# tturturiello/lightweight-snappy

Measured on AMD Instinct MI355X. Metric: compress + decompress MB/s at 1/2/4/8 MI355X; % HBM roofline; ratio vs ref, higher is better.
Workload: dtype u8

## Files before the change

### lightweight-snappy_amd/csrc/snappy_kernels.hip

```cpp
#include <hip/hip_runtime.h>
#include <stdint.h>
#include <type_traits>

#include "snappy_kernels.h"

#ifndef SNAPPY_TU
#define SNAPPY_TU 0
#endif
#define SNAPPY_TU_COMPRESS (SNAPPY_TU != 2)
#define SNAPPY_TU_DECODE (SNAPPY_TU != 1)

#if ((defined(SNAPPY_K2_NOLIT) && SNAPPY_K2_NOLIT) || defined(SNAPPY_K4_NOFAR)) && !defined(SNAPPY_MEASUREMENT_BUILD)
#error "SNAPPY_K2_NOLIT / SNAPPY_K4_NOFAR write wrong output: measurement builds only (-DSNAPPY_MEASUREMENT_BUILD)"
#endif

namespace snappy_amd {

__device__ int amdgcn_writelane(int val, int lanesel, int old) __asm("llvm.amdgcn.writelane.i32");


constexpr uint32_t kTable = 4096;
constexpr uint32_t kMul = 0x1e35a7bdu;

typedef uint32_t u32x4 __attribute__((ext_vector_type(4)));
// ... 390 lines not shown
    })

    uint32_t T = 256, lg = 8;
    while (T < kTable && T < L) { T <<= 1; lg++; }
    const uint32_t shift = 32 - lg;

    const uint32_t cur0 = __builtin_amdgcn_readfirstlane(REG_OF(0));
    const uint32_t init = TAG_OF(cur0) << 16;
    for (uint32_t i = lane; i < kTable; i += 64) TBL_WRITE(i, init);
    __syncthreads();

    uint32_t *tok = reinterpret_cast<uint32_t *>(tokens) + (uint64_t)u * tok_cap;
    uint32_t *tok_full = reinterpret_cast<uint32_t *>(tokens) + ((uint64_t)gridDim.x + u) * tok_cap;
    uint32_t tka = 0, tkb = 0;
    uint32_t nt = 0, pend = 0;
    uint32_t acc = 0, cend = 0;
    if (hdr_mode == SNAPPY_HDR_EVERY_UNIT) acc = varint_len(L);
    else if (hdr_mode == SNAPPY_HDR_FIRST_UNIT && u == 0) acc = varint_len(header_value);
    uint32_t *const segu = seg_off + 2 * (uint64_t)u * segs;
    auto flush_tokens = [&]() {
        const bool has = lane < pend;
        const uint32_t pos = tka & 0xFFFF, len = tka >> 16, end = pos + len;
        const uint32_t prev = (uint32_t)__builtin_amdgcn_update_dpp((int)cend, (int)end, 0x138, 0xF, 0xF, false);
        const uint32_t litn = pos - prev;
        if (has) {
            const uint32_t lc = len - 4 < 255 ? len - 4 : 255u, gc = litn < 255 ? litn : 255u;
            tok[nt + lane] = tkb | (lc << 16) | (gc << 24);
            if (lc == 255 || gc == 255) tok_full[nt + lane] = litn | (len << 16);
        }
        const uint32_t b = has ? (litn ? literal_bytes(litn) : 0u) + copy_bytes(len, tkb) : 0u;
        uint32_t tot;
        const uint32_t ex = wave_excl_scan(b, lane, &tot);
        if (has && ((nt + lane) & (kK2Seg - 1)) == 0)
            *reinterpret_cast<uint2 *>(segu + 2 * ((nt + lane) / kK2Seg)) = make_uint2(acc + ex, prev);
        if (pend) cend = __builtin_amdgcn_readlane(end, pend - 1);
        acc += tot;
        nt += pend;
        pend = 0;
    };

    uint32_t q0 = 0, d0 = 0, dr = 0, dv = 0, bv = 0, hv = 0;
    uint32_t pdl1 = 0, pdc = 0;
    uint16_t ent = 0;
    uint8_t ent_t = 0;
    uint32_t adr = 0, word = 0;
    uint32_t pdnz = 0;
    uint64_t m_win = 0, m_win17 = 0;
    bool lsw = false;
#ifndef SNAPPY_K1R_WIN_ALIGN
#define SNAPPY_K1R_WIN_ALIGN 1
#endif
#define WINDOW_AT(qq)                                                                              \
    do {                                                                                           \
        q0 = (qq);                                                                                 \
        ring_to((q0 >> 8) + 2, std::true_type{});     \
        d0 = q0 >> 2;                                                                              \
        dr = d0 & 63;                                                                              \
        {                                                                                          \
            uint32_t _r0, _r1;                                                                     \
            REG_PAIR(d0 >> 6, _r0, _r1);                                                           \
            dv = lane >= dr ? _r0 : _r1;                                                           \
        }                                                                                          \
        if (SNAPPY_K1R_WIN_ALIGN == 2 || (SNAPPY_K1R_WIN_ALIGN && !BIG)) { \
                          \
                                \
            const uint32_t _p = q0 + lane;                                                          \
            const uint32_t _k = (_p - 1) >> 2;                        \
            const uint32_t _a = (uint32_t)__builtin_amdgcn_ds_bpermute((int)(_k << 2), (int)dv);   \
            const uint32_t _b = (uint32_t)__builtin_amdgcn_ds_bpermute((int)((_k + 1) << 2), (int)dv); \
            bv = __builtin_amdgcn_alignbit(_a, _b, 0u - (_p << 3));                                  \
        } else {                                                                                   \
            const uint32_t _k = d0 + (((q0 & 3) + lane) >> 2);      \
            const uint32_t _a = (uint32_t)__builtin_amdgcn_ds_bpermute((int)(_k << 2), (int)dv);   \
            const uint32_t _b = (uint32_t)__builtin_amdgcn_ds_bpermute((int)((_k + 1) << 2), (int)dv); \
            bv = funnel_bytes(_a, _b, perm_sel((q0 + lane) & 3));                                 \
        }                                                                                          \
        {                                                                                          \
            const uint32_t _pr = bv * kMul;                                                        \
            hv = (_pr >> shift) | (__builtin_amdgcn_ubfe(_pr, shift - 8, 8) << 16);                \
        }                                                                                          \
    } while (0)
#define WINDOW_LS(qq)                                                                              \
    do {                                                                                           \
        WINDOW_AT(qq);                                                                             \
        adr = TBL_ADR(hv & 0xFFFF);                                                                \
        TBL_READ_ENT(adr);                              \
                          \
        const uint32_t _best = nearest_same_key<DMAX>(__builtin_amdgcn_alignbit(hv, hv, 16) + 0x10000u); \
        const bool _has = _best < 65536u;                                                          \
        const uint32_t _pd = _has ? _best >> 8 : 0u;                                               \
              \
        pdl1 = _has ? lane - _pd + 1 - (_pd == 1 ? 1u : 0u) : 0xFFFFFF00u;  \
        pdc = q0 + lane - _pd;                                                                     \
        pdnz = _best & 0xFFu;              \
                   \
        const int32_t _w16 = (int32_t)(L - 16 - q0), _w17 = (int32_t)(L - 17 - q0);              \
        const bool _inw = (int32_t)lane <= _w16 && lane <= 62;                                     \
        m_win = __ballot(_inw);                                                                    \
        m_win17 = __ballot((int32_t)lane <= _w17 && lane <= 62);                                   \
        word = (q0 + lane) | (hv & 0xFF0000u);                                                     \
        if (!_inw) word |= 1u << 24;    \
        lsw = true;                                                      \
    } while (0)

    auto match_len_from = [&](uint32_t pf, uint32_t cand, uint32_t len) -> uint32_t {
            for (;;) {
                if (pf + len >= L) break;
                const uint32_t qa = pf + len, qb = cand + len;
                ring_to((qa >> 8) + 2, std::false_type{});
                const uint32_t a0 = DW_LANES(qa >> 2), b0 = CAND_LANES(qb >> 2);
                const uint32_t va = funnel_bytes(a0, wave_shl1(a0), perm_sel(qa & 3));
                const uint32_t vb = funnel_bytes(b0, wave_shl1(b0), perm_sel(qb & 3));
                const uint32_t yy = lane < 63 ? (va ^ vb) : 0;
                const uint64_t bb = __ballot(yy != 0);
                if (bb) {
                    const uint32_t m = (uint32_t)__builtin_ctzll(bb);
                    len += 4 * m + ((uint32_t)__builtin_clz(__builtin_amdgcn_readlane(yy, m)) >> 3);
                    break;
                }
                len += 252;
            }
        return len;
    };
    auto match_len = [&](uint32_t pf, uint32_t cand) -> uint32_t {
        const uint32_t pa = (uint32_t)__builtin_amdgcn_ds_bpermute((int)(((pf >> 2) + lane) << 2), (int)dv);
        const uint32_t ca = CAND_LANES(cand >> 2);
        const uint32_t pv = funnel_bytes(pa, wave_shl1(pa), perm_sel(pf & 3));
        const uint32_t cv = funnel_bytes(ca, wave_shl1(ca), perm_sel(cand & 3));
        const uint32_t y = pv ^ cv;
        const uint64_t bad = __ballot(y != 0) & 0xFFFFull;
        if (bad) {
            const uint32_t m = (uint32_t)__builtin_ctzll(bad);
            return 4 * m + ((uint32_t)__builtin_clz(__builtin_amdgcn_readlane(y, m)) >> 3);
        }
        return match_len_from(pf, cand, 64);
    };
    auto put_token = [&](uint32_t pf, uint32_t len, uint32_t off) {
        tka = (uint32_t)amdgcn_writelane((int)(pf | (len << 16)), (int)pend, (int)tka);
        tkb = (uint32_t)amdgcn_writelane((int)off, (int)pend, (int)tkb);
        pend++;
    };
    uint32_t dka = 0, dkb = 0, dkn = 0;
    auto drain_token = [&]() {
        tka = (uint32_t)amdgcn_writelane((int)dka, (int)pend, (int)tka);
        tkb = (uint32_t)amdgcn_writelane((int)dkb, (int)pend, (int)tkb);
        pend += dkn;
        dkn = 0;
    };

#ifdef SNAPPY_K1R_RSTAMPS
    const uint64_t t_loop = clock64();
    uint64_t rs_flush = 0, rs_win = 0, rs_asm = 0;
    uint32_t rs_n = 0, rs_nfl = 0, rs_nasm = 0, rs_code[6] = {0, 0, 0, 0, 0, 0};
#endif
#ifdef SNAPPY_K1R_STATS
    const uint64_t t_loop = clock64();
    uint32_t n_probe = 0, n_match = 0, n_round = 0, n_refresh = 0;
#endif

#if !defined(SNAPPY_K1R_STATS) && !defined(SNAPPY_K1R_LSTAMPS) && !defined(SNAPPY_K1R_CXX_ROUNDS)
#define K1R_ASM_ROUNDS 1
#else
#define K1R_ASM_ROUNDS 0
#endif
#if K1R_ASM_ROUNDS
#ifndef SNAPPY_K1R_PAD32
#define SNAPPY_K1R_PAD32 2
#endif
#ifndef SNAPPY_K1R_PAD64
#define SNAPPY_K1R_PAD64 0
#endif
#ifndef SNAPPY_K1R_PAD64A
#define SNAPPY_K1R_PAD64A -1
#endif
#ifndef SNAPPY_K1R64_HALF32
#define SNAPPY_K1R64_HALF32 1
#endif
#define K1R_STR2(x) #x
#define K1R_STR(x) K1R_STR2(x)
#define K1R_LOOP_PLACE(pad) ".if " K1R_STR(pad) " >= 0\n.p2align 6\n.rept " K1R_STR(pad) "\ns_nop 0\n.endr\n.endif\n"
#define K1R_CAND32 "s_lshr_b32 %[s0], %[c], 8\n\t"
#define K1R_CAND64                                                                                  \
    "s_cmp_lt_u32 %[c], %[seghi]\n\t"                                                              \
    "s_cbranch_scc1 L%=_far\n\t"                                                                   \
    "s_bfe_u32 %[s0], %[c], 0x70008\n\t"                                                           \
    "s_cmp_eq_u32 %[s0], 127\n\t"                                                                  \
    "s_cbranch_scc1 L%=_wrap\n\t"
#define K1R_SEGHI64(seg_hi) "s"(((seg_hi) - kRegs) << 8)
#define K1R_HIT_PREDTAG                                                                             \
    "v_cndmask_b32_sdwa %[t1], %[pdc], %[ent], vcc dst_sel:DWORD dst_unused:UNUSED_PAD "             \
    "src0_sel:DWORD src1_sel:WORD_0\n\t"                           \
    "v_cndmask_b32_e32 %[t0], %[pdnz], %[entt], vcc\n\t"                           \
    "v_cmp_eq_u32_sdwa %[hm], %[t0], %[word] src0_sel:DWORD src1_sel:WORD_1\n\t"
#define K1R_HIT32 K1R_HIT_PREDTAG
#define K1R_HIT64 K1R_HIT_PREDTAG
#define K1R_DRAIN                                                                                   \
    "s_mov_b32 m0, %[pend]\n\t"           \
    "v_writelane_b32 %[tka], %[dka], m0\n\t"                                                        \
    "v_writelane_b32 %[tkb], %[dkb], m0\n\t"                                                        \
    "s_add_u32 %[pend], %[pend], %[dkn]\n\t"
#define K1R_SKIPFIX "s_cmp_eq_u32 %[dkn], 0\n\ts_cselect_b32 %[skip], %[skip], 32\n\t"
#define K1R_INSERTS(cnt, lo)                                                                        \
    "s_bfm_b64 exec, " cnt ", " lo "\n\t"                                                          \
    "ds_write_b16 %[adr], %[word]\n\t"                                                              \
    "ds_write_b8_d16_hi %[adrt], %[word] offset:%[tagb]\n\t"                                        \
    "s_mov_b64 exec, %[sx]\n\t"                                                                     \
    "ds_read_u16 %[ent], %[adr]\n\t"                                   \
    "ds_read_u8 %[entt], %[adrt] offset:%[tagb]\n\t"
#ifndef SNAPPY_K1R_X45
#define SNAPPY_K1R_X45 1
#endif
#if SNAPPY_K1R_X45
#define K1R_LENCHECK                                                                                \
    "v_readlane_b32 %[s0], %[t2], %[s1]\n\t"                                                        \
    "s_add_u32 %[s2], %[s0], -4\n\t"                                                                \
    "s_cmp_gt_u32 %[s2], 59\n\t"                                                                    \
    "s_cbranch_scc1 L%=_x4\n\t"
#define K1R_X4 "s_cmp_lt_u32 %[s0], 4\n\ts_cbranch_scc1 L%=_x5\n\ts_mov_b32 %[code], 4\n\ts_branch L%=_end\n"
#else
#define K1R_LENCHECK                                                                                \
    "s_cmp_gt_u32 %[s1], 15\n\t"                                                                    \
    "s_cbranch_scc1 L%=_x4\n\t"                                                                    \
    "v_readlane_b32 %[s0], %[t2], %[s1]\n\t"                                                       \
    "s_cmp_lt_u32 %[s0], 4\n\t"            \
    "s_cbranch_scc1 L%=_x5\n\t"
#define K1R_X4 "s_mov_b32 %[code], 4\n\ts_branch L%=_end\n"
#endif
#define K1R_NOHIT_TAIL(T)                                                                           \
    "s_cmp_gt_u32 %[skip], %[lsmax]\n\t"                                                           \
    "s_cbranch_scc1 L%=_x1\n\t"                                                                    \
    "s_cmp_gt_u32 %[p], %[lm16]\n\t"                                                               \
    "s_cbranch_scc1 L%=_x1\n\t"                                                                    \
    "s_cmp_gt_u32 %[lane0], %[l0max]\n\t"                                                          \
    "s_cbranch_scc1 L%=_x2\n\t"                                                                    \
    "s_cmp_le_u32 %[skip], %[skipmax]\n\t"                                                         \
    "s_cbranch_scc1 L%=_top" T "\n"
#ifndef SNAPPY_K1R_EARLY_DK
#define SNAPPY_K1R_EARLY_DK 1
#endif
#if SNAPPY_K1R_EARLY_DK
#define K1R_DK_EARLY "s_sub_u32 %[dkb], %[pf], %[c]\n\t"
#define K1R_DK_LATE "s_mov_b32 %[dkn], 1\n\t"
#else
#define K1R_DK_EARLY
#define K1R_DK_LATE "s_sub_u32 %[dkb], %[pf], %[c]\n\ts_mov_b32 %[dkn], 1\n\t"
#endif
#define K1R_ROUND_BODY(CAND, HIT, T)                                                                \
            "L%=_top" T ":\n\t"                                                                          \
            "s_lshl_b64 %[valid], %[dmask], %[lane0]\n\t"                                           \
            "v_cmp_gt_i32_e32 vcc, %[lane0], %[pdl1]\n\t"                   \
            "s_waitcnt lgkmcnt(0)\n\t"                                                              \
            HIT                                                                                     \
            "s_and_b64 %[hm], %[hm], %[valid]\n\t"                                                  \
            "s_cbranch_scc0 L%=_nohit" T "\n\t"                                      \
            "s_ff1_i32_b64 %[f], %[hm]\n\t"                                                         \
            "v_readlane_b32 %[c], %[t1], %[f]\n\t"                                                  \
            "s_add_u32 %[pf], %[q0], %[f]\n\t"                                                      \
            "v_add3_u32 %[t2], %[pf], -1, %[lane4]\n\t"               \
            "ds_bpermute_b32 %[t2], %[t2], %[dv]\n\t"                         \
            CAND                                                                                    \
            "s_bfe_u32 %[s1], %[c], 0x60002\n\t"                                                    \
            "v_cmp_le_u32_e32 vcc, %[s1], %[lane]\n\t"            \
            "v_add_u32_e32 %[t1], %[c], %[lane4]\n\t"                                               \
            "s_set_gpr_idx_on %[s0], gpr_idx(SRC0,SRC1)\n\t"                                        \
            "v_cndmask_b32_e32 %[t3], v3, v2, vcc\n\t"                                              \
            "s_set_gpr_idx_off\n\t"                                                                 \
            "ds_bpermute_b32 %[t3], %[t1], %[t3]\n\t"                          \
            "L%=_farret" T ":\n\t"                                                                       \
            K1R_DRAIN                          \
            K1R_DK_EARLY                                                                            \
            "s_cmp_lt_u32 %[lane0], %[f]\n\t"                                                       \
            "s_subb_u32 %[s0], %[lane0], 0\n\t"                                            \
            "v_mul_i32_i24_e64 %[t0], %[pf], -8\n\t"                         \
            "s_sub_u32 %[s2], %[f], %[s0]\n\t"                                                      \
            "s_add_u32 %[s2], %[s2], 1\n\t"                              \
            "s_and_b32 %[s3], %[c], 3\n\t"                                                          \
            "s_mul_i32 %[s3], %[s3], 0xfefefeff\n\t"                                                \
            "s_add_i32 %[s3], %[s3], 0x7060504\n\t"                         \
            "s_waitcnt lgkmcnt(0)\n\t"                                                \
            "v_mov_b32_dpp %[t1], %[t2] wave_shl:1 row_mask:0xf bank_mask:0xf bound_ctrl:1\n\t"     \
            "v_mov_b32_dpp %[t4], %[t3] wave_shl:1 row_mask:0xf bank_mask:0xf bound_ctrl:1\n\t"     \
            "v_alignbit_b32 %[t2], %[t2], %[t1], %[t0]\n\t"                                         \
            "v_perm_b32 %[t3], %[t3], %[t4], %[s3]\n\t"                                             \
            K1R_INSERTS("%[s2]", "%[s0]")                                                           \
            "v_cmp_ne_u32_e32 vcc, %[t2], %[t3]\n\t"                                                \
            "v_xor_b32_e32 %[t2], %[t2], %[t3]\n\t"                                                 \
            "v_ffbh_u32_e32 %[t2], %[t2]\n\t"                                                       \
            "v_bfe_u32 %[t2], %[t2], 3, 2\n\t"                                                      \
            "v_lshl_or_b32 %[t2], %[lane], 2, %[t2]\n\t"  \
            "s_ff1_i32_b32 %[s1], vcc_lo\n\t"                                                       \
            K1R_LENCHECK                                                                            \
            "s_add_u32 %[lane0], %[f], %[s0]\n\t"                                                   \
            "s_pack_ll_b32_b16 %[dka], %[pf], %[s0]\n\t"                                           \
            K1R_DK_LATE                                                                             \
            "s_cmp_le_i32 %[lane0], %[lim0]\n\t"          \
            "s_cbranch_scc1 L%=_top" T "\n\t"                                                            \
            "s_sub_u32 %[s2], %[L], %[pf]\n\t"  \
            "s_min_u32 %[s0], %[s0], %[s2]\n\t"                                                     \
            "s_add_u32 %[p], %[pf], %[s0]\n\t"                                                      \
            "s_sub_u32 %[lane0], %[p], %[q0]\n\t"                                                   \
            "s_lshl_b32 %[s1], %[s0], 16\n\t"                                                       \
            "s_or_b32 %[dka], %[s1], %[pf]\n\t"                                                     \
            "s_cmp_gt_u32 %[p], %[lm16]\n\t"                                                        \
            "s_cbranch_scc1 L%=_x1\n\t"                                                             \
            "s_branch L%=_x2\n"                                                                     \
            "L%=_nohit" T ":\n\t"                                                                        \
            K1R_SKIPFIX                                                                             \
            "s_and_b64 %[valid], %[valid], %[mwin]\n\t"                                             \
            "s_bcnt1_i32_b64 %[s0], %[valid]\n\t"  \
            K1R_DRAIN                                                                               \
            "s_mov_b32 %[dkn], 0\n\t"                                                               \
            "s_add_i32 %[s1], %[lane0], -1\n\t"                                                     \
            "s_add_u32 %[s2], %[skip], %[s0]\n\t"                                                   \
            "s_add_i32 %[s3], %[s2], -1\n\t"                                                        \
            "s_add_u32 %[c], %[s0], 1\n\t"                           \
            K1R_INSERTS("%[c]", "%[s1]")                     \
            "s_lshr_b32 %[s3], %[s3], 5\n\t"              \
            "s_add_u32 %[lane0], %[s1], %[s0]\n\t"           \
            "s_add_u32 %[lane0], %[lane0], %[s3]\n\t"                                               \
            "s_add_u32 %[p], %[q0], %[lane0]\n\t"                                                   \
            "s_mov_b32 %[skip], %[s2]\n\t"                                                          \
            K1R_NOHIT_TAIL(T)
#if SNAPPY_K1R64_HALF32
#define K1R64_HALF_SEL "s_cmp_eq_u32 %[seghi], 0\n\ts_cbranch_scc1 L%=_topa\n"
#define K1R64_HALF_LOOP "s_branch L%=_x3\n" K1R_LOOP_PLACE(SNAPPY_K1R_PAD64A) K1R_ROUND_BODY(K1R_CAND32, K1R_HIT64, "a")
#else
#define K1R64_HALF_SEL ""
#define K1R64_HALF_LOOP ""
#endif
#define K1R_ASM_ROUNDS_STMT(code, fx, cx, e32, et32, CAND, SEGHI, HIT, PAD, DUAL_SEL, DUAL_LOOP)    \
    do {                                                                                            \
        uint32_t _m0s, _pf, _s0, _s1, _s2, _s3, _t0, _t1, _t2, _t3, _t4;                            \
        uint64_t _valid, _hm;                                                                       \
        asm volatile(                                                                               \
            "s_mov_b32 %[m0s], m0\n\t"                                                              \
            "s_cmp_gt_u32 %[skip], %[skipmax]\n\t"    \
            "s_cbranch_scc1 L%=_x3\n"                                                               \
            DUAL_SEL                                                                                \
            K1R_LOOP_PLACE(PAD)                                                                     \
            K1R_ROUND_BODY(CAND, HIT, "")                                                           \
            DUAL_LOOP                                                                               \
            "L%=_x3:\n\ts_mov_b32 %[code], 3\n\ts_branch L%=_end\n"                                 \
            "L%=_x1:\n\ts_mov_b32 %[code], 1\n\ts_branch L%=_end\n"                                 \
            "L%=_x2:\n\ts_mov_b32 %[code], 2\n\ts_branch L%=_end\n"                                 \
            "L%=_x4:\n\t" K1R_X4                                                                   \
            "L%=_far:\n\t"                     \
            "s_and_b32 %[s1], %[c], -4\n\t"                                                         \
            "v_add_u32_e32 %[t1], %[s1], %[lane4]\n\t"                                              \
            "global_load_dword %[t3], %[t1], %[srcb]\n\t"                                           \
            "s_mov_b32 %[s1], 0x10203\n\t"                                                          \
            "s_waitcnt vmcnt(0)\n\t"                                                                \
            "v_perm_b32 %[t3], %[t3], %[t3], %[s1]\n\t"     \
            "s_branch L%=_farret\n"                                                                 \
            "L%=_wrap:\n\t"                \
            "s_bfe_u32 %[s1], %[c], 0x60002\n\t"                                                    \
            "v_cmp_le_u32_e32 vcc, %[s1], %[lane]\n\t"                                              \
            "v_add_u32_e32 %[t1], %[c], %[lane4]\n\t"                                               \
            "s_nop 0\n\t"                                                                            \
            "v_cndmask_b32_e32 %[t3], v2, v129, vcc\n\t"                                            \
            "ds_bpermute_b32 %[t3], %[t1], %[t3]\n\t"                                               \
            "s_branch L%=_farret\n"                                                                 \
            "L%=_x5:\n\ts_mov_b32 %[code], 5\n"                                                     \
            "L%=_end:\n\t"                                                                          \
            K1R_SKIPFIX                                                                             \
            "s_mov_b32 m0, %[m0s]\n\t"                                                              \
            "s_waitcnt lgkmcnt(0)"                                                                  \
            : [p] "+s"(p), [skip] "+s"(skip), [lane0] "+s"(lane0), [pend] "+s"(pend), [dka] "+s"(dka), \
              [dkb] "+s"(dkb), [dkn] "+s"(dkn), [code] "=&s"(code), [f] "=&s"(fx),                     \
              [c] "=&s"(cx),                                                                        \
              [m0s] "=&s"(_m0s), [pf] "=&s"(_pf), [s0] "=&s"(_s0), [s1] "=&s"(_s1), [s2] "=&s"(_s2),   \
              [s3] "=&s"(_s3), [valid] "=&s"(_valid), [hm] "=&s"(_hm), [ent] "+v"(e32),                \
              [entt] "+v"(et32), [tka] "+v"(tka), [tkb] "+v"(tkb), [t0] "=&v"(_t0), [t1] "=&v"(_t1),  \
              [t2] "=&v"(_t2), [t3] "=&v"(_t3), [t4] "=&v"(_t4)                                        \
            : [q0] "s"(q0), [L] "s"(L), [lm16] "s"(L - 16), [mwin] "s"(m_win), [seghi] SEGHI,         \
              [lim0] "s"(__builtin_elementwise_min((int32_t)(62 - SNAPPY_K1R_RMIN), (int32_t)L - 16 - (int32_t)q0)), \
              [dv] "v"(dv),                                                                         \
              [pdl1] "v"(pdl1), [pdc] "v"(pdc), [pdnz] "v"(pdnz), [adr] "v"(adr), [adrt] "v"(adr >> 1), \
              [word] "v"(word), [lane] "v"(lane), [lane4] "v"(lane << 2), [srcb] "s"(src),            \
              [sx] "s"(__builtin_amdgcn_read_exec()),      \
              [skipmax] "i"(64 - DMAX), [dmask] "i"((1u << DMAX) - 1), [lsmax] "i"(64 - SNAPPY_K1R_LSMIN), \
              [l0max] "i"(62 - SNAPPY_K1R_RMIN), [tagb] "i"(kTagBase), "{v[2:33]}"(g0), "{v[34:65]}"(g1), \
              "{v[66:97]}"(g2), "{v[98:129]}"(g3)                                                      \
            : "vcc", "scc", "memory");                                                              \
    } while (0)
#endif
#if defined(SNAPPY_K1R_LSTAMPS)
    uint64_t seg[6] = {0, 0, 0, 0, 0, 0};
    uint64_t s0, s1, s2, s3, s4, s5, s6;
#endif
    uint32_t p = 1, skip = 33;
    while (!(L - p < (skip >> 5) + 15)) {
#ifdef SNAPPY_K1R_STATS
        n_round++;
#endif
        if (skip <= 64 - SNAPPY_K1R_LSMIN) {
            auto refresh = [&]() {
                LSTAMP(s5);
#ifdef SNAPPY_K1R_STATS
                n_refresh++;
#endif
#ifdef SNAPPY_K1R_RSTAMPS
                uint64_t r0, r1, r2;
                const bool rfl = pend + dkn > 48;
                if constexpr (BIG) {
                    RSTAMP(r0);
                    WINDOW_LS(p - 1);
                    RSTAMP(r1);
                    if (rfl) flush_tokens();
                    RSTAMP(r2);
                    rs_win += r1 - r0;
                    rs_flush += r2 - r1;
                } else {
                    RSTAMP(r0);
                    if (rfl) flush_tokens();
                    RSTAMP(r1);
                    WINDOW_LS(p - 1);
                    RSTAMP(r2);
                    rs_flush += r1 - r0;
                    rs_win += r2 - r1;
                }
                rs_n++;
                rs_nfl += rfl;
                if (false)
#endif
                if constexpr (BIG) {
                    const bool fl = pend + dkn > 48;
                    WINDOW_LS(p - 1);
                    if (fl) flush_tokens();
                } else
                {
                    if (pend + dkn > 48) flush_tokens();
                    WINDOW_LS(p - 1);
                }
                LSTAMP(s6);
                LSEG(5, s5, s6);
            };
            uint32_t lane0 = p - q0;
            bool went = false;
            if (!lsw || lane0 + SNAPPY_K1R_RMIN > 62) {
                refresh();
                lane0 = 1;
                went = true;
            }
            if (!went) TBL_READ_ENT(adr);
            for (;;) {
#if K1R_ASM_ROUNDS
                {
                    uint32_t code, fx, cx;
                    uint32_t e32 = ent, et32 = ent_t;
#ifdef SNAPPY_K1R_RSTAMPS
                    uint64_t ra0, ra1;
                    RSTAMP(ra0);
#endif
                    if constexpr (BIG)
                        K1R_ASM_ROUNDS_STMT(code, fx, cx, e32, et32, K1R_CAND64, K1R_SEGHI64(seg_hi), K1R_HIT64, SNAPPY_K1R_PAD64,
                                            K1R64_HALF_SEL, K1R64_HALF_LOOP);
                    else
                        K1R_ASM_ROUNDS_STMT(code, fx, cx, e32, et32, K1R_CAND32, "i"(0), K1R_HIT32, SNAPPY_K1R_PAD32, "", "");
#ifdef SNAPPY_K1R_RSTAMPS
                    RSTAMP(ra1);
                    rs_asm += ra1 - ra0;
                    rs_nasm++;
                    rs_code[code < 6 ? code : 0]++;
#endif
                    ent = (uint16_t)e32;
                    ent_t = (uint8_t)et32;
                    if (code == 1) break;
                    if (code == 2) {
                        refresh();
                        lane0 = 1;
                        continue;
                    }
                    if (code >= 4) {
                        const uint32_t f = fx, pf = q0 + fx, c = cx;
                        uint32_t np;
                        if (code == 4) {
                            uint32_t len = __builtin_elementwise_min(match_len_from(pf, c, 64), L - pf);
                            dka = pf | (len << 16);
                            dkb = pf - c;
                            dkn = 1;
                            np = pf + len;
                            skip = 32;
                        } else {
                            dkn = 0;
                            if (f == lane0) {
                                TBL_INSERT(lane - (lane0 - 1) <= 1);
                                LDS_ORDER();
                                TBL_READ_ENT(adr);
                            }
                            np = pf + ((skip + f - lane0) >> 5);
                            skip += f - lane0 + 1;
                        }
                        p = np;
                        if (!(skip <= 64 - SNAPPY_K1R_LSMIN && p <= L - 16)) break;
                        lane0 = p - q0;
                        if (lane0 + SNAPPY_K1R_RMIN > 62) {
                            refresh();
                            lane0 = 1;
                        }
                        continue;
                    }
                }
#endif
                LSTAMP(s0);
                drain_token();
                uint64_t valid = (((1ull << DMAX) - 1) << lane0) & m_win;
                if (__builtin_expect(skip > 64 - DMAX, 0)) {
                    const uint32_t kcap = 64 - skip;
                    valid = ((2ull << kcap) - 1) << lane0;
                    if (lane0 + kcap < 64) valid &= ~((1ull << (lane0 + kcap)) & ~m_win17);
                    valid &= m_win;
                }
                const bool inr = (int32_t)pdl1 >= (int32_t)lane0;
                const uint32_t hitnz = (inr ? pdnz : (uint32_t)ent_t) ^ ((word >> 16) & 0xFFu);
                const uint64_t hm = __ballot(hitnz == 0) & valid;
                const uint32_t candv = inr ? pdc : ent;
                const uint32_t f = (uint32_t)__builtin_ctzll(hm);
                LSTAMP(s1);
                LSEG(0, s0, s1);
                uint32_t np;
                if (__builtin_expect(hm != 0, 1)) {
                    const uint32_t pf = q0 + f;
                    const uint32_t c = __builtin_amdgcn_readlane(candv, f) & 0xFFFF;
                    const uint32_t pa = (uint32_t)__builtin_amdgcn_ds_bpermute(
                        (int)(((pf >> 2) + lane) << 2), (int)dv);
                    const uint32_t ca = CAND_LANES(c >> 2);
                    __builtin_amdgcn_sched_barrier(0);
                    const uint32_t lo0 = f > lane0 ? lane0 - 1 : lane0;
                    TBL_INSERT(lane - lo0 <= f - lo0);
                    LDS_ORDER();
                    TBL_READ_ENT(adr);
                    LSTAMP(s2);
                    LSEG(1, s1, s2);
                    const uint32_t pv = funnel_bytes(pa, wave_shl1(pa), perm_sel(pf & 3));
                    const uint32_t cv = funnel_bytes(ca, wave_shl1(ca), perm_sel(c & 3));
                    const uint32_t y = pv ^ cv;
                    const uint64_t bad = __ballot(y != 0) & 0xFFFFull;
                    const uint32_t lenv = 4 * lane + ((uint32_t)__builtin_clz(y | 1) >> 3);
                    uint32_t len = __builtin_amdgcn_readlane(lenv, (uint32_t)__builtin_ctzll(bad) & 63);
                    if (__builtin_expect(bad == 0, 0)) len = match_len_from(pf, c, 64);
                    LSTAMP(s3);
                    LSEG(2, s2, s3);
#ifdef SNAPPY_K1R_STATS
                    n_probe += f - lane0 + 1;
#endif
                    len = __builtin_elementwise_min(len, L - pf);
                    dka = pf | (len << 16);
                    dkb = pf - c;
                    if (__builtin_expect(len >= 4, 1)) {
#ifdef SNAPPY_K1R_STATS
                        n_match++;
#endif
                        dkn = 1;
                        np = pf + len;
                        skip = 32;
                    } else {
                        dkn = 0;
                        if (f == lane0) {
                            TBL_INSERT(lane - (lane0 - 1) <= 1);
                            LDS_ORDER();
                            TBL_READ_ENT(adr);
                        }
                        np = pf + ((skip + f - lane0) >> 5);
                        skip += f - lane0 + 1;
                    }
                } else {
                    LSTAMP(s3);
                    dka = dkb = dkn = 0;
                    const uint32_t nk = (uint32_t)__builtin_popcountll(valid);
                    TBL_INSERT(lane - (lane0 - 1) <= nk);
                    LDS_ORDER();
                    TBL_READ_ENT(adr);
                    np = q0 + lane0 + nk - 1 + ((skip + nk - 1) >> 5);
                    skip += nk;
#ifdef SNAPPY_K1R_STATS
                    n_probe += nk;
#endif
                }
                p = np;
                LSTAMP(s4);
                LSEG(3, s3, s4);
                LSEG(4, s0, s4);
#ifdef SNAPPY_K1R_STATS
                n_round++;
#endif
                if (__builtin_expect(!(skip <= 64 - SNAPPY_K1R_LSMIN && p <= L - 16), 0)) break;
                lane0 = p - q0;
                if (__builtin_expect(lane0 + SNAPPY_K1R_RMIN > 62, 0)) {
                    refresh();
                    lane0 = 1;
                }
            }
            drain_token();
#ifdef SNAPPY_K1R_STATS
            n_round--;
#endif
            continue;
        }
#ifdef SNAPPY_K1R_STATS
        if constexpr (!BIG) n_farc++;
#endif
        lsw = false;
        if (p - 1 < q0 || p + 12 > q0 + 64) WINDOW_AT(p - 1);
        const uint32_t sk = skip + lane;
        const uint32_t pk = p + skipsum(sk) - skipsum(skip);
        const uint32_t bend = (sk >> 5) + 15;
        const uint32_t inval = (uint32_t)(((int32_t)(W - 1 - lane)) >> 31) |
                               (uint32_t)(((int32_t)(L - pk) - (int32_t)bend) >> 31) |
                               (uint32_t)(((int32_t)(q0 + 64) - (int32_t)(pk + 12)) >> 31);
        const uint32_t ik = inval ? 1 : pk - q0;
        const uint32_t hvp = (uint32_t)__builtin_amdgcn_ds_bpermute((int)(ik << 2), (int)hv);
        const uint32_t hvq = (uint32_t)__builtin_amdgcn_ds_bpermute((int)((ik - 1) << 2), (int)hv);
        const uint32_t h = hvp & 0xFFFF, a = hvq & 0xFFFF;
        const uint32_t e = TBL_READ(h);
        const uint32_t notdup = ~eqm(((sk - 1) >> 5) ^ 1);
        const uint32_t conflict = tconf<W>(h, a, notdup) & ~eqm(lane);
        const uint32_t hit = TAG_EQ(e, hvp) ? 0xFFFFFFFFu : 0u;
        const uint64_t stop = __ballot((inval | conflict | hit) != 0);
        const uint32_t f = (uint32_t)__builtin_ctzll(stop);
        if (lane < f) {
            TBL_WRITE(a, (pk - 1) | (hvq & 0xFFFF0000u));
            TBL_WRITE(h, pk | (hvp & 0xFFFF0000u));
        }
        LDS_ORDER();
        const uint64_t hits = __ballot((hit & ~(inval | conflict)) != 0);
#ifdef SNAPPY_K1R_STATS
        n_probe += f + ((hits >> f) & 1);
#endif
        uint32_t next_f = f;
        if ((hits >> f) & 1) {
            const uint32_t pf = __builtin_amdgcn_readlane(pk, f);
            const uint32_t cand = __builtin_amdgcn_readlane(e, f) & 0xFFFF;
            const uint32_t hf = __builtin_amdgcn_readlane(hvp, f);
            uint32_t len = match_len(pf, cand);
            if (len >= 4) {
                if (len > L - pf) len = L - pf;
#ifdef SNAPPY_K1R_STATS
                n_match++;
#endif
                if (pend == 64) flush_tokens();
                put_token(pf, len, pf - cand);
                TBL_WRITE(hf & 0xFFFF, pf | (hf & 0xFFFF0000u));
                LDS_ORDER();
                skip = 32;
                p = pf + len;
                continue;
            }
            const uint32_t af = __builtin_amdgcn_readlane(hvq, f);
            TBL_WRITE(af & 0xFFFF, (pf - 1) | (af & 0xFFFF0000u));
            TBL_WRITE(hf & 0xFFFF, pf | (hf & 0xFFFF0000u));
            LDS_ORDER();
            next_f = f + 1;
        }
        p = skip + next_f <= 64 ? p + next_f : p + skipsum(skip + next_f) - skipsum(skip);
        skip += next_f;
    }
#undef WINDOW_AT
#undef WINDOW_LS
#undef TAG_OF
#undef TBL_READ
#undef TBL_WRITE
#undef TBL_READ3
#undef TBL_WRITE3
#undef TBL_ADR
#undef TBL_READ_ENT
#undef TBL_INSERT
#undef TAG_EQ
#undef LDS_ORDER
#undef CAND_LANES
#undef K1R_COUNT
    if constexpr (BIG) asm volatile("s_waitcnt vmcnt(0)" ::: "memory");
    flush_tokens();
    if (lane == 0) {
        if ((nt & (kK2Seg - 1)) == 0) *reinterpret_cast<uint2 *>(segu + 2 * (nt / kK2Seg)) = make_uint2(acc, cend);
        ntok_out[u] = nt;
        sizes[u] = acc + (L > cend ? literal_bytes(L - cend) : 0u);
    }
#ifdef SNAPPY_K1R_RSTAMPS
    if (lane == 0) {
        uint64_t *st = reinterpret_cast<uint64_t *>(tokens + (uint64_t)gridDim.x * tok_cap) + 4 * (uint64_t)u;
        st[0] = clock64() - t_loop;
        st[1] = rs_flush | (rs_asm << 24);
        st[2] = rs_win | ((uint64_t)rs_nasm << 40);
        st[3] = rs_n | ((uint64_t)rs_nfl << 16) | ((uint64_t)rs_code[3] << 32) | ((uint64_t)(rs_code[4] + rs_code[5]) << 48);
    }
#endif
#ifdef SNAPPY_K1R_STATS
    if (lane == 0) {
        uint64_t *st = reinterpret_cast<uint64_t *>(tokens + (uint64_t)gridDim.x * tok_cap) + 4 * (uint64_t)u;
        st[0] = clock64() - t_loop;
#if defined(SNAPPY_K1R_LSTAMPS)
        st[1] = seg[0] | (seg[1] << 32);
        st[3] = seg[2] | (seg[3] << 32);
        st[2] = seg[4] | (seg[5] << 32);
#else
        st[1] = n_farc | ((uint64_t)n_reload << 32);
        st[2] = n_probe | ((uint64_t)n_round << 32);
        st[3] = n_match | ((uint64_t)n_refresh << 32);
#endif
    }
#endif
}

#if SNAPPY_TU_COMPRESS
__global__ __launch_bounds__(64, 3) void k1r_match_units(const uint8_t *__restrict__ in, uint64_t n, uint32_t unit,
                                                          uint32_t hdr_mode, uint64_t header_value,
                                                          uint2 *__restrict__ tokens, uint32_t tok_cap,
                                                          uint32_t *__restrict__ ntok_out,
                                                          uint32_t *__restrict__ sizes,
                                                          uint32_t *__restrict__ seg_off, uint32_t segs)
{
    k1r_body<false>(in, n, unit, hdr_mode, header_value, tokens, tok_cap, ntok_out, sizes, seg_off, segs);
}
#endif

#if SNAPPY_TU_COMPRESS
__global__ __launch_bounds__(64, 3) void k1r_match_units64(const uint8_t *__restrict__ in, uint64_t n, uint32_t unit,
                                                            uint32_t hdr_mode, uint64_t header_value,
                                                            uint2 *__restrict__ tokens, uint32_t tok_cap,
                                                            uint32_t *__restrict__ ntok_out,
                                                            uint32_t *__restrict__ sizes,
                                                            uint32_t *__restrict__ seg_off, uint32_t segs)
{
    k1r_body<true>(in, n, unit, hdr_mode, header_value, tokens, tok_cap, ntok_out, sizes, seg_off, segs);
}
#endif

__device__ __forceinline__ uint32_t wave_excl_scan32(uint32_t v, uint32_t *total)
{
    uint32_t x = v;
    x += dpp0<0x111, 0xF>(x);
    x += dpp0<0x112, 0xF>(x);
    x += dpp0<0x114, 0xF>(x);
    x += dpp0<0x118, 0xF>(x);
    x += dpp0<0x142, 0xA>(x);
    *total = (uint32_t)__builtin_amdgcn_readlane((int)x, 31);
    return x - v;
}

template <typename P>
__device__ __forceinline__ void put_copy(P *o, uint32_t len, uint32_t off)
{
    while (len > 68) {
        o[0] = 0xFE; o[1] = (uint8_t)off; o[2] = (uint8_t)(off >> 8);
        o += 3; len -= 64;
    }
    if (len > 64) {
        o[0] = 0xEE; o[1] = (uint8_t)off; o[2] = (uint8_t)(off >> 8);
        o += 3; len -= 60;
    }
    if (len < 12 && off < 2048) {
        o[0] = (uint8_t)((((off >> 8) << 5) + ((len - 4) << 2) + 1));
        o[1] = (uint8_t)off;
    } else {
        o[0] = (uint8_t)(((len - 1) << 2) | 2); o[1] = (uint8_t)off; o[2] = (uint8_t)(off >> 8);
    }
}

template <typename P>
__device__ __forceinline__ void put_element(P *w, const uint8_t *__restrict__ src, uint32_t s0, uint32_t litn,
                                            uint32_t hl, uint32_t len, uint32_t off, bool wide_ok)
{
    if (hl == 1) w[0] = (uint8_t)((litn - 1) << 2);
    else if (hl == 2) { w[0] = 60 << 2; w[1] = (uint8_t)(litn - 1); }
    else if (hl == 3) { w[0] = 61 << 2; w[1] = (uint8_t)(litn - 1); w[2] = (uint8_t)((litn - 1) >> 8); }
    if (litn <= 16) {
        if (wide_ok) {
            const uintptr_t sa = reinterpret_cast<uintptr_t>(src + s0);
            const uint32_t sh = (uint32_t)(sa & 3);
            const uint32_t *aw = reinterpret_cast<const uint32_t *>(sa - sh);
            const uint32_t d0 = aw[0], d1 = aw[1], d2 = aw[2], d3 = aw[3], d4 = aw[4];
            const uint32_t r[4] = {__builtin_amdgcn_alignbyte(d1, d0, sh), __builtin_amdgcn_alignbyte(d2, d1, sh),
                                   __builtin_amdgcn_alignbyte(d3, d2, sh), __builtin_amdgcn_alignbyte(d4, d3, sh)};
#pragma unroll
            for (uint32_t j = 0; j < 16; j++)
                if (j < litn) w[hl + j] = (uint8_t)(r[j >> 2] >> (8 * (j & 3)));
        } else {
            for (uint32_t j = 0; j < litn; j++) w[hl + j] = src[s0 + j];
        }
    }
    if (len) put_copy(w + hl + litn, len, off);
}

#ifndef SNAPPY_K2_STAGE
#define SNAPPY_K2_STAGE 4096
#endif
constexpr uint32_t kK2Stage = SNAPPY_K2_STAGE;

__device__ __forceinline__ void put_element_lds(__attribute__((address_space(3))) uint8_t *stage, uint32_t at,
                                                const uint8_t *__restrict__ src, uint32_t s0, uint32_t litn,
                                                uint32_t hl, uint32_t len, uint32_t off, bool wide_ok, bool live,
                                                uint32_t lane, const uint32_t *lw, uint32_t sh)
{
    const uint32_t dum = kK2Stage + 4 + 4 * lane;
#define K2_ST8(cond, adr, v) stage[(cond) ? (adr) : dum] = (uint8_t)(v)
    const uint32_t lm1 = litn - 1;
    K2_ST8(live && hl >= 1, at, hl == 1 ? lm1 << 2 : (hl == 2 ? 60u << 2 : 61u << 2));
    K2_ST8(live && hl >= 2, at + 1, lm1);
    K2_ST8(live && hl == 3, at + 2, lm1 >> 8);
    const uint32_t lp = at + hl;
    if (litn <= 16) {
        if (wide_ok) {
            const uint32_t r0 = __builtin_amdgcn_alignbyte(lw[1], lw[0], sh), r1 = __builtin_amdgcn_alignbyte(lw[2], lw[1], sh);
            const uint32_t r2 = __builtin_amdgcn_alignbyte(lw[3], lw[2], sh), r3 = __builtin_amdgcn_alignbyte(lw[4], lw[3], sh);
#define K2_ST32(k, r) *(__attribute__((address_space(3))) u32u *)(stage + (live && 4 * (k) + 4 <= litn ? lp + 4 * (k) : dum)) = (r)
            K2_ST32(0, r0); K2_ST32(1, r1); K2_ST32(2, r2); K2_ST32(3, r3);
#undef K2_ST32
            const uint32_t fb = litn & ~3u, rem = litn & 3u;
            const uint32_t rt = fb == 0 ? r0 : (fb == 4 ? r1 : (fb == 8 ? r2 : r3));
            K2_ST8(live && rem > 0, lp + fb, rt);
            K2_ST8(live && rem > 1, lp + fb + 1, rt >> 8);
            K2_ST8(live && rem > 2, lp + fb + 2, rt >> 16);
        } else if (live) {
            for (uint32_t j = 0; j < litn; j++) stage[lp + j] = src[s0 + j];
        }
    }
    const uint32_t cp = lp + litn;
    if (len <= 64) {
        const bool c1 = len < 12 && off < 2048;
        const bool has = live && len != 0;
        K2_ST8(has, cp, c1 ? (((off >> 8) << 5) + ((len - 4) << 2) + 1) : (((len - 1) << 2) | 2));
        K2_ST8(has, cp + 1, off);
        K2_ST8(has && !c1, cp + 2, off >> 8);
    } else if (live) {
        put_copy(stage + cp, len, off);
    }
#undef K2_ST8
}

__device__ __forceinline__ void k2_long_literals(__attribute__((address_space(3))) uint8_t *w,
                                                 const uint8_t *__restrict__ src, uint64_t longs, uint32_t litn,
                                                 uint32_t s0v, uint32_t d0v, uint32_t lane)
{
    while (longs) {
        const uint32_t k = (uint32_t)__builtin_ctzll(longs);
        longs &= longs - 1;
// ... 1732 lines not shown
```

Baseline: 72780.

## Rebuild the match window inside the asm round loop instead of exiting

In the 32-bit (non-BIG) compress path, the hand-written asm round loop no longer returns with code 2 when the window runs out. It now rebuilds the next 64-byte window in place: it gathers the data words via gpr indexing and bpermute, hashes, reads the hash table, and recomputes the pending-match prefix scan with DPP steps, then jumps back to the loop top. This saves the round trip through compiler-generated C++ code and the asm re-entry setup for each window. In exchange, much more state is passed in and out of the asm block as read-write operands, which adds register pressure. The fixed code is only valid for DMAX 13, and m_win17 has to be recomputed in the skip-cap path. Extra RSTAMPS counters are also added for profiling.

New measurement: 76850, median of 6. 1.06x the previous value.

```diff
diff --git a/lightweight-snappy_amd/csrc/snappy_kernels.hip b/lightweight-snappy_amd/csrc/snappy_kernels.hip
--- a/lightweight-snappy_amd/csrc/snappy_kernels.hip
+++ b/lightweight-snappy_amd/csrc/snappy_kernels.hip
@@ -566,6 +566,9 @@
     const uint64_t t_loop = clock64();
     uint64_t rs_flush = 0, rs_win = 0, rs_asm = 0;
     uint32_t rs_n = 0, rs_nfl = 0, rs_nasm = 0, rs_code[6] = {0, 0, 0, 0, 0, 0};
+    uint64_t rs_gout = 0, rs_gin = 0, rs_ra1 = 0, rs_r2 = 0;
+    uint32_t rs_ng = 0;
+    bool rs_c2 = false, rs_gopen = false;
 #endif
 #ifdef SNAPPY_K1R_STATS
     const uint64_t t_loop = clock64();
@@ -646,7 +649,7 @@
     "s_cmp_gt_u32 %[p], %[lm16]\n\t"                                                               \
     "s_cbranch_scc1 L%=_x1\n\t"                                                                    \
     "s_cmp_gt_u32 %[lane0], %[l0max]\n\t"                                                          \
-    "s_cbranch_scc1 L%=_x2\n\t"                                                                    \
+    "s_cbranch_scc1 L%=_win\n\t"                                                                    \
     "s_cmp_le_u32 %[skip], %[skipmax]\n\t"                                                         \
     "s_cbranch_scc1 L%=_top" T "\n"
 #ifndef SNAPPY_K1R_EARLY_DK
@@ -717,7 +720,7 @@
             "s_or_b32 %[dka], %[s1], %[pf]\n\t"                                                     \
             "s_cmp_gt_u32 %[p], %[lm16]\n\t"                                                        \
             "s_cbranch_scc1 L%=_x1\n\t"                                                             \
-            "s_branch L%=_x2\n"                                                                     \
+            "s_branch L%=_win\n"                                                                    \
             "L%=_nohit" T ":\n\t"                                                                        \
             K1R_SKIPFIX                                                                             \
             "s_and_b64 %[valid], %[valid], %[mwin]\n\t"                                             \
@@ -742,7 +745,94 @@
 #define K1R64_HALF_SEL ""
 #define K1R64_HALF_LOOP ""
 #endif
-#define K1R_ASM_ROUNDS_STMT(code, fx, cx, e32, et32, CAND, SEGHI, HIT, PAD, DUAL_SEL, DUAL_LOOP)    \
+#ifndef SNAPPY_K1R_WIN_INLOOP
+#define SNAPPY_K1R_WIN_INLOOP 1
+#endif
+#define K1R_WIN_NONE "L%=_win:\n"
+#define K1R_WIN_STEP(dst)                                                                           \
+    "v_add_u32_dpp %[t1], %[t1], %[pdl1] wave_shr:1 row_mask:0xf bank_mask:0xf bound_ctrl:1\n\t"    \
+    "v_bitop3_b32 " dst ", %[t0], %[t1], %[s0] bitop3:0x6c\n\t"
+#define K1R_WIN_PAIR                                                                                \
+    K1R_WIN_STEP("%[t4]")                                                                           \
+    "s_nop 0\n\t"                                                                                   \
+    K1R_WIN_STEP("%[pdc]")                                                                          \
+    "v_min3_u32 %[pdnz], %[pdnz], %[t4], %[pdc]\n\t"
+#define K1R_WIN_PATH                                                                                \
+    "L%=_win:\n\t"                                                                                  \
+    K1R_SKIPFIX                                                                                     \
+    "s_add_u32 %[s0], %[pend], %[dkn]\n\t"                                                          \
+    "s_cmp_gt_u32 %[s0], 48\n\t"                         \
+    "s_cbranch_scc1 L%=_x2\n\t"                                                                     \
+    "s_add_u32 %[q0], %[p], -1\n\t"                                                                 \
+    "s_lshr_b32 %[s0], %[q0], 8\n\t"                                                                \
+    "s_bfe_u32 %[s1], %[q0], 0x60002\n\t"                                                   \
+    "s_set_gpr_idx_on %[s0], gpr_idx(SRC0)\n\t"                                                     \
+    "v_mov_b32_e32 %[t0], v2\n\t"                                                                   \
+    "v_mov_b32_e32 %[t1], v3\n\t"                                                                   \
+    "s_set_gpr_idx_off\n\t"                                                                         \
+    "v_cmp_gt_u32_e32 vcc, %[s1], %[lane]\n\t"                  \
+    "v_add_u32_e32 %[t2], %[q0], %[lane]\n\t"                                                       \
+    "v_mul_i32_i24_e64 %[t3], %[t2], -8\n\t"                         \
+    "v_add_u32_e32 %[t4], -1, %[t2]\n\t"                                                            \
+    "v_cndmask_b32_e32 %[dv], %[t0], %[t1], vcc\n\t"                                                \
+    "v_and_b32_e32 %[t4], -4, %[t4]\n\t"                               \
+    "ds_bpermute_b32 %[t0], %[t4], %[dv]\n\t"                                                       \
+    "ds_bpermute_b32 %[t1], %[t4], %[dv] offset:4\n\t"                                              \
+    "s_mov_b32 %[s0], 0xffff0000\n\t"                                                               \
+    "s_mov_b32 %[s2], 0xff0000\n\t"                                                                 \
+    "s_sub_i32 %[s1], %[lm16], %[q0]\n\t"                                          \
+    "s_min_i32 %[lim0], %[s1], %[l0max]\n\t"                                                        \
+    "s_min_i32 %[s1], %[s1], 62\n\t"                                       \
+    "s_mov_b32 %[lane0], 1\n\t"                                                                     \
+    "v_mov_b32_e32 %[pdl1], 0x100\n\t"                                                              \
+    "s_waitcnt lgkmcnt(0)\n\t"                                                                      \
+    "v_alignbit_b32 %[t0], %[t0], %[t1], %[t3]\n\t"                          \
+    "v_mul_lo_u32 %[t0], %[t0], %[kmul]\n\t"                                                        \
+    "v_lshrrev_b32_e32 %[adrt], %[shift], %[t0]\n\t"                                  \
+    "v_bfe_u32 %[t3], %[t0], %[sh8], 8\n\t"                                            \
+    "v_lshlrev_b32_e32 %[adr], 1, %[adrt]\n\t"                                                      \
+    "v_lshl_or_b32 %[hv], %[t3], 16, %[adrt]\n\t"                                                   \
+    "ds_read_u16 %[ent], %[adr]\n\t"                                  \
+    "ds_read_u8 %[entt], %[adrt] offset:%[tagb]\n\t"                                                \
+    "v_alignbit_b32 %[t0], %[hv], %[hv], 16\n\t"                                                    \
+    "v_add_u32_e32 %[t0], 0x10000, %[t0]\n\t"                       \
+    "v_cmp_ge_i32_e32 vcc, %[s1], %[lane]\n\t"             \
+    "v_and_or_b32 %[word], %[hv], %[s2], %[t2]\n\t"                                                 \
+    "s_mov_b64 %[mwin], vcc\n\t"                                                                    \
+    "v_add_u32_dpp %[t1], %[t0], %[pdl1] wave_shr:1 row_mask:0xf bank_mask:0xf bound_ctrl:1\n\t"    \
+    "v_bitop3_b32 %[pdnz], %[t0], %[t1], %[s0] bitop3:0x6c\n\t"                                     \
+    "v_or_b32_e32 %[t3], 0x1000000, %[word]\n\t"                                                    \
+    K1R_WIN_STEP("%[t4]")                                                                           \
+    "v_cndmask_b32_e32 %[word], %[t3], %[word], vcc\n\t"                   \
+    K1R_WIN_STEP("%[pdc]")                                                                          \
+    "v_min3_u32 %[pdnz], %[pdnz], %[t4], %[pdc]\n\t"                                                \
+    K1R_WIN_PAIR K1R_WIN_PAIR K1R_WIN_PAIR K1R_WIN_PAIR K1R_WIN_PAIR         \
+    "v_lshrrev_b32_e32 %[t3], 8, %[pdnz]\n\t"                                     \
+    "v_cmp_gt_u32_e32 vcc, 0x10000, %[pdnz]\n\t"                        \
+    "v_cmp_eq_u32_e64 %[hm], 1, %[t3]\n\t"                                                          \
+    "v_and_b32_e32 %[pdnz], 0xff, %[pdnz]\n\t"                                                      \
+    "v_add_u32_e32 %[t1], 1, %[lane]\n\t"                                                           \
+    "v_mov_b32_e32 %[t4], 0xffffff00\n\t"                                                           \
+    "v_subb_co_u32_e64 %[t1], %[hm], %[t1], %[t3], %[hm]\n\t"        \
+    "v_cndmask_b32_e32 %[t3], 0, %[t3], vcc\n\t"                                                    \
+    "v_cndmask_b32_e32 %[pdl1], %[t4], %[t1], vcc\n\t"                                              \
+    "v_sub_u32_e32 %[pdc], %[t2], %[t3]\n\t"                                                        \
+    "s_cmp_gt_u32 %[skip], %[skipmax]\n\t"                         \
+    "s_cbranch_scc1 L%=_x3\n\t"                                                                     \
+    "s_branch L%=_top\n"
+static_assert(SNAPPY_K1R_DMAX == 13 || !SNAPPY_K1R_WIN_INLOOP, "K1R_WIN_PATH is written out for DMAX 13");
+#define K1R_WINOPS_NONE_OUT
+#define K1R_WINOPS_NONE_IN(SEGHI)                                                                   \
+    [q0] "s"(q0), [L] "s"(L), [lm16] "s"(L - 16), [mwin] "s"(m_win), [seghi] SEGHI,                 \
+    [lim0] "s"(__builtin_elementwise_min((int32_t)(62 - SNAPPY_K1R_RMIN), (int32_t)L - 16 - (int32_t)q0)), \
+    [dv] "v"(dv), [pdl1] "v"(pdl1), [pdc] "v"(pdc), [pdnz] "v"(pdnz), [adr] "v"(adr), [adrt] "v"(adr >> 1), \
+    [word] "v"(word),
+#define K1R_WINOPS_PATH_OUT                                                                         \
+    , [q0] "+s"(q0), [mwin] "+s"(m_win), [lim0] "+s"(lim0), [dv] "+v"(dv), [hv] "+v"(hv), [pdl1] "+v"(pdl1), \
+      [pdc] "+v"(pdc), [pdnz] "+v"(pdnz), [adr] "+v"(adr), [adrt] "+v"(adrt), [word] "+v"(word)
+#define K1R_WINOPS_PATH_IN(SEGHI)                                                                   \
+    [L] "s"(L), [lm16] "s"(L - 16), [seghi] SEGHI, [shift] "s"(shift), [sh8] "s"(shift - 8), [kmul] "s"(kMul),
+#define K1R_ASM_ROUNDS_STMT(code, fx, cx, e32, et32, CAND, SEGHI, HIT, PAD, DUAL_SEL, DUAL_LOOP, WIN, WIN_OUT, WIN_IN) \
     do {                                                                                            \
         uint32_t _m0s, _pf, _s0, _s1, _s2, _s3, _t0, _t1, _t2, _t3, _t4;                            \
         uint64_t _valid, _hm;                                                                       \
@@ -756,6 +846,7 @@
             DUAL_LOOP                                                                               \
             "L%=_x3:\n\ts_mov_b32 %[code], 3\n\ts_branch L%=_end\n"                                 \
             "L%=_x1:\n\ts_mov_b32 %[code], 1\n\ts_branch L%=_end\n"                                 \
+            WIN                                                                                     \
             "L%=_x2:\n\ts_mov_b32 %[code], 2\n\ts_branch L%=_end\n"                                 \
             "L%=_x4:\n\t" K1R_X4                                                                   \
             "L%=_far:\n\t"                     \
@@ -785,12 +876,9 @@
               [m0s] "=&s"(_m0s), [pf] "=&s"(_pf), [s0] "=&s"(_s0), [s1] "=&s"(_s1), [s2] "=&s"(_s2),   \
               [s3] "=&s"(_s3), [valid] "=&s"(_valid), [hm] "=&s"(_hm), [ent] "+v"(e32),                \
               [entt] "+v"(et32), [tka] "+v"(tka), [tkb] "+v"(tkb), [t0] "=&v"(_t0), [t1] "=&v"(_t1),  \
-              [t2] "=&v"(_t2), [t3] "=&v"(_t3), [t4] "=&v"(_t4)                                        \
-            : [q0] "s"(q0), [L] "s"(L), [lm16] "s"(L - 16), [mwin] "s"(m_win), [seghi] SEGHI,         \
-              [lim0] "s"(__builtin_elementwise_min((int32_t)(62 - SNAPPY_K1R_RMIN), (int32_t)L - 16 - (int32_t)q0)), \
-              [dv] "v"(dv),                                                                         \
-              [pdl1] "v"(pdl1), [pdc] "v"(pdc), [pdnz] "v"(pdnz), [adr] "v"(adr), [adrt] "v"(adr >> 1), \
-              [word] "v"(word), [lane] "v"(lane), [lane4] "v"(lane << 2), [srcb] "s"(src),            \
+              [t2] "=&v"(_t2), [t3] "=&v"(_t3), [t4] "=&v"(_t4) WIN_OUT                                \
+            : WIN_IN(SEGHI)                                                                         \
+              [lane] "v"(lane), [lane4] "v"(lane << 2), [srcb] "s"(src),                              \
               [sx] "s"(__builtin_amdgcn_read_exec()),      \
               [skipmax] "i"(64 - DMAX), [dmask] "i"((1u << DMAX) - 1), [lsmax] "i"(64 - SNAPPY_K1R_LSMIN), \
               [l0max] "i"(62 - SNAPPY_K1R_RMIN), [tagb] "i"(kTagBase), "{v[2:33]}"(g0), "{v[34:65]}"(g1), \
@@ -833,6 +921,13 @@
                     rs_flush += r1 - r0;
                     rs_win += r2 - r1;
                 }
+                rs_gopen = rs_c2 && !rfl;
+                if (rs_gopen) {
+                    rs_gout += r0 - rs_ra1;
+                    rs_r2 = r2;
+                    rs_ng++;
+                }
+                rs_c2 = false;
                 rs_n++;
                 rs_nfl += rfl;
                 if (false)
@@ -865,17 +960,30 @@
 #ifdef SNAPPY_K1R_RSTAMPS
                     uint64_t ra0, ra1;
                     RSTAMP(ra0);
-#endif
-                    if constexpr (BIG)
+                    if (rs_gopen) rs_gin += ra0 - rs_r2;
+                    rs_gopen = false;
+#endif
+                    if constexpr (BIG) {
                         K1R_ASM_ROUNDS_STMT(code, fx, cx, e32, et32, K1R_CAND64, K1R_SEGHI64(seg_hi), K1R_HIT64, SNAPPY_K1R_PAD64,
-                                            K1R64_HALF_SEL, K1R64_HALF_LOOP);
-                    else
-                        K1R_ASM_ROUNDS_STMT(code, fx, cx, e32, et32, K1R_CAND32, "i"(0), K1R_HIT32, SNAPPY_K1R_PAD32, "", "");
+                                            K1R64_HALF_SEL, K1R64_HALF_LOOP, K1R_WIN_NONE, K1R_WINOPS_NONE_OUT, K1R_WINOPS_NONE_IN);
+                    } else {
+#if SNAPPY_K1R_WIN_INLOOP
+                        int32_t lim0 = __builtin_elementwise_min((int32_t)(62 - SNAPPY_K1R_RMIN), (int32_t)L - 16 - (int32_t)q0);
+                        uint32_t adrt = adr >> 1;
+                        K1R_ASM_ROUNDS_STMT(code, fx, cx, e32, et32, K1R_CAND32, "i"(0), K1R_HIT32, SNAPPY_K1R_PAD32, "", "",
+                                            K1R_WIN_PATH, K1R_WINOPS_PATH_OUT, K1R_WINOPS_PATH_IN);
+#else
+                        K1R_ASM_ROUNDS_STMT(code, fx, cx, e32, et32, K1R_CAND32, "i"(0), K1R_HIT32, SNAPPY_K1R_PAD32, "", "",
+                                            K1R_WIN_NONE, K1R_WINOPS_NONE_OUT, K1R_WINOPS_NONE_IN);
+#endif
+                    }
 #ifdef SNAPPY_K1R_RSTAMPS
                     RSTAMP(ra1);
                     rs_asm += ra1 - ra0;
                     rs_nasm++;
                     rs_code[code < 6 ? code : 0]++;
+                    rs_ra1 = ra1;
+                    rs_c2 = code == 2;
 #endif
                     ent = (uint16_t)e32;
                     ent_t = (uint8_t)et32;
@@ -922,7 +1030,12 @@
                 if (__builtin_expect(skip > 64 - DMAX, 0)) {
                     const uint32_t kcap = 64 - skip;
                     valid = ((2ull << kcap) - 1) << lane0;
-                    if (lane0 + kcap < 64) valid &= ~((1ull << (lane0 + kcap)) & ~m_win17);
+                    uint64_t mw17 = m_win17;
+#if K1R_ASM_ROUNDS && SNAPPY_K1R_WIN_INLOOP
+                    if constexpr (!BIG)
+                        mw17 = __ballot((int32_t)lane <= (int32_t)(L - 17 - q0) && lane <= 62);
+#endif
+                    if (lane0 + kcap < 64) valid &= ~((1ull << (lane0 + kcap)) & ~mw17);
                     valid &= m_win;
                 }
                 const bool inr = (int32_t)pdl1 >= (int32_t)lane0;
@@ -1093,9 +1206,9 @@
 #ifdef SNAPPY_K1R_RSTAMPS
     if (lane == 0) {
         uint64_t *st = reinterpret_cast<uint64_t *>(tokens + (uint64_t)gridDim.x * tok_cap) + 4 * (uint64_t)u;
-        st[0] = clock64() - t_loop;
+        st[0] = (clock64() - t_loop) | (rs_gout << 30) | ((uint64_t)rs_ng << 52);
         st[1] = rs_flush | (rs_asm << 24);
-        st[2] = rs_win | ((uint64_t)rs_nasm << 40);
+        st[2] = rs_win | (rs_gin << 24) | ((uint64_t)rs_nasm << 46);
         st[3] = rs_n | ((uint64_t)rs_nfl << 16) | ((uint64_t)rs_code[3] << 32) | ((uint64_t)(rs_code[4] + rs_code[5]) << 48);
     }
 #endif
```
